# ZKI-PH-ImageAnalysis/seq2squiggle

Hardware: AMD Instinct MI355X
Metric: signal samples/sec at 5 kb reads (padded [chunks x 250] samples the predict path emits) (higher is better)
Workload: dtype f16x3

## Files before the change

### seq2squiggle_amd/csrc/s2s_device_h.h

```cpp
#pragma once
#include "s2s_device.h"

typedef _Float16 h8 __attribute__((ext_vector_type(8)));
typedef _Float16 h4 __attribute__((ext_vector_type(4)));

static constexpr float S2S_SHIFT_BIAS = 2.0f;
#define S2S_PF_FLOATS (1024 + 16 + 16)
#define S2S_Z2_FLOATS (256 + 64)
#define S2S_PROG_INTS 16
#define S2S_SV_FLOATS 960
#define WS_ADVP(n, bit) (ws += ((S2S_ABL & (bit)) ? 0 : (n)))
#ifndef S2S_NO_SB_ATT
#define SB_ATT() __builtin_amdgcn_sched_barrier(0)
#else
#define SB_ATT()
#endif
#ifndef S2S_NO_SB_GEMM
#define SB_GEMM() __builtin_amdgcn_sched_barrier(0)
#else
#define SB_GEMM()
#endif
#define MFMAH(a, b, c) __builtin_amdgcn_mfma_f32_16x16x32_f16((a), (b), (c), 0, 0, 0)
#ifndef S2S_MFMA_SPLIT
#define S2S_MFMA_SPLIT 0
// ... 5 lines not shown

__device__ __forceinline__ h8 as_h8(const f32x4 v) { return __builtin_bit_cast(h8, v); }

typedef _Float16 h2v __attribute__((ext_vector_type(2)));
template <bool LO = true>
__device__ __forceinline__ void split2(const float a, const float b, const float one, unsigned& hi, unsigned& lo) {
    unsigned hb = __builtin_bit_cast(unsigned, (h2v{(_Float16)a, (_Float16)b}));
    if (!LO) { hi = hb; lo = 0u; return; }
    asm("" : "+v"(hb));
    const h2v h = __builtin_bit_cast(h2v, hb);
    const h2v l = {(_Float16)__builtin_fmaf(a, one, -(float)h[0]), (_Float16)__builtin_fmaf(b, one, -(float)h[1])};
    hi = hb;
    lo = __builtin_bit_cast(unsigned, l);
}
template <bool LO = true>
__device__ __forceinline__ void exp_split4(const f32x4 s, const float one, unsigned& h0, unsigned& h1, unsigned& l0,
                                           unsigned& l1) {
    const float e0 = (S2S_ABL & 1) ? s[0] : __builtin_amdgcn_exp2f(s[0]), e1 = (S2S_ABL & 1) ? s[1] : __builtin_amdgcn_exp2f(s[1]);
    const float e2 = (S2S_ABL & 1) ? s[2] : __builtin_amdgcn_exp2f(s[2]), e3 = (S2S_ABL & 1) ? s[3] : __builtin_amdgcn_exp2f(s[3]);
    if (S2S_ABL & 2) {
        h0 = __float_as_uint(e0); l0 = __float_as_uint(e1); h1 = __float_as_uint(e2); l1 = __float_as_uint(e3);
        return;
    }
    split2<LO>(e0, e1, one, h0, l0);
    split2<LO>(e2, e3, one, h1, l1);
}
typedef unsigned uv4 __attribute__((ext_vector_type(4)));
typedef unsigned uv2 __attribute__((ext_vector_type(2)));
template <bool LO = true>
__device__ __forceinline__ HL split8(const f32x4 t0, const f32x4 t1, const float one) {
    unsigned h0, h1, h2, h3, l0, l1, l2, l3;
    split2<LO>(t0[0], t0[1], one, h0, l0);
    split2<LO>(t0[2], t0[3], one, h1, l1);
    split2<LO>(t1[0], t1[1], one, h2, l2);
    split2<LO>(t1[2], t1[3], one, h3, l3);
    HL o;
    o.hi = __builtin_bit_cast(h8, (uv4{h0, h1, h2, h3}));
    o.lo = __builtin_bit_cast(h8, (uv4{l0, l1, l2, l3}));
    return o;
}
template <bool LO = true>
__device__ __forceinline__ void split4(const f32x4 t, const float one, h4& hi, h4& lo) {
    unsigned h0, h1, l0, l1;
    split2<LO>(t[0], t[1], one, h0, l0);
    split2<LO>(t[2], t[3], one, h1, l1);
    hi = __builtin_bit_cast(h4, (uv2{h0, h1}));
    lo = __builtin_bit_cast(h4, (uv2{l0, l1}));
}

template <bool NATURAL = false>
__host__ __device__ constexpr int att32_key_at(const int p) {
    return NATURAL ? p : 16 * ((((p & 63) >> 2) - ((p >> 6) & 1)) & 15) + 4 * (p >> 6) + (p & 3);
}
template <int TV, bool NATURAL = false>
__device__ __forceinline__ void att32_mask_tile(f32x16& t, const int tile, const int h) {
#pragma unroll
    for (int r = 0; r < 16; ++r) {
        const int row = (r & 3) + 8 * (r >> 2);
        const bool p0 = att32_key_at<NATURAL>(32 * tile + row) >= TV, p1 = att32_key_at<NATURAL>(32 * tile + row + 4) >= TV;
        if (p0 && p1) t[r] = -__builtin_inff();
        else if (p1) t[r] = h ? -__builtin_inff() : t[r];
        else if (p0) t[r] = h ? t[r] : -__builtin_inff();
    }
}

template <int NQ, int WAVES, int NKT = 16> struct AttnLdsH {
    static_assert(NQ == 2 && NKT == 16, "the 32x32x16 attention core: 32 queries per wave, 256 keys");
    static constexpr int KEYS = 16 * NKT;
    static constexpr int K_BYTES = 8 * 2 * KEYS * 8 * 2;
    static constexpr int VS = KEYS + 8;
    static constexpr int V_BYTES = 8 * 16 * VS * 2;
    static constexpr int C_ROWS = 3;
    static constexpr int C_BYTES = C_ROWS * VS * 2;
    static constexpr int Q_WAVE_BYTES = NQ * 2 * 2 * 16 * 8 * 2;
    static constexpr int BYTES = K_BYTES + V_BYTES + C_BYTES + WAVES * Q_WAVE_BYTES;
};

template <int NQ, bool LO = true>
__device__ __forceinline__ void mm_unit_h(f32x4 (&acc)[NQ], const f32x4 (&f)[4], const HL (&x)[NQ][2]) {
#pragma unroll
    for (int kb = 0; kb < 2; ++kb) {
        const h8 wh = as_h8(f[2 * kb]), wl = as_h8(f[2 * kb + 1]);
#pragma unroll
        for (int q = 0; q < NQ; ++q) acc[q] = MFMAH(wh, x[q][kb].hi, acc[q]);
        if (LO) {
#pragma unroll
            for (int q = 0; q < NQ; ++q) acc[q] = MFMAH(wh, x[q][kb].lo, acc[q]);
#pragma unroll
            for (int q = 0; q < NQ; ++q) acc[q] = MFMAH(wl, x[q][kb].hi, acc[q]);
        }
    }
}

template <int NQ, bool LO = true>
__device__ __forceinline__ void mm_unit_h_t(f32x4 (&acc)[NQ], const f32x4 (&f)[4], const HL (&x)[NQ][2]) {
#pragma unroll
    for (int kb = 0; kb < 2; ++kb) {
        const h8 wh = as_h8(f[2 * kb]), wl = as_h8(f[2 * kb + 1]);
#pragma unroll
        for (int q = 0; q < NQ; ++q) acc[q] = MFMAH(x[q][kb].hi, wh, acc[q]);
        if (LO) {
#pragma unroll
            for (int q = 0; q < NQ; ++q) acc[q] = MFMAH(x[q][kb].lo, wh, acc[q]);
#pragma unroll
            for (int q = 0; q < NQ; ++q) acc[q] = MFMAH(x[q][kb].hi, wl, acc[q]);
        }
    }
}

template <int NQ>
__device__ __forceinline__ void linear64_h(const float* __restrict__ wu, const float* __restrict__ bias, int lane,
                                           const HL (&xb)[NQ][2], f32x4 (&y)[NQ][4]) {
    const int g = lane >> 4;
#pragma unroll
    for (int mt = 0; mt < 4; ++mt) {
        f32x4 f[4], t[NQ];
        load_unit(f, wu + mt * 1024 + lane * 4);
        const f32x4 b = ldg4(bias + 16 * mt + 4 * g);
// ... 11 lines not shown
    return fmaxf(__uint_as_float(t[0]), __uint_as_float(t[1]));
}
__device__ __forceinline__ float sum_h(float v) {
    const unsigned u = __float_as_uint(v);
    auto t = __builtin_amdgcn_permlane32_swap(u, u, false, false);
    return __uint_as_float(t[0]) + __uint_as_float(t[1]);
}
struct SelA { h8 a[2]; };
__device__ __forceinline__ SelA split_selectors(const int h) {
    const int row = threadIdx.x & 31, rho = row & 15;
    const int j = (rho & 3) + 4 * (rho >> 3);
    const unsigned w = (((rho >> 2) & 1) == h) ? ((j & 1) ? 0xBC000000u : 0x0000BC00u) : 0u;
    uv4 sel;
#pragma unroll
    for (int d = 0; d < 4; ++d) sel[d] = (j >> 1) == d ? w : 0u;
    const uv4 z = {0u, 0u, 0u, 0u};
    SelA o;
    o.a[0] = __builtin_bit_cast(h8, row < 16 ? sel : z);
    o.a[1] = __builtin_bit_cast(h8, row < 16 ? z : sel);
    return o;
}
template <bool LO>
__device__ __forceinline__ void pv_split_mfma(f32x16 sc, const h8 (&va)[2], const SelA& sel, f32x16& O) {
    unsigned hw[8];
#pragma unroll
    for (int r = 0; r < 16; ++r) sc[r] = __builtin_amdgcn_exp2f(sc[r]);
#pragma unroll
    for (int p = 0; p < 8; ++p) hw[p] = __builtin_bit_cast(unsigned, (h2v{(_Float16)sc[2 * p], (_Float16)sc[2 * p + 1]}));
    const h8 hb0 = __builtin_bit_cast(h8, (uv4{hw[0], hw[1], hw[2], hw[3]})), hb1 = __builtin_bit_cast(h8, (uv4{hw[4], hw[5], hw[6], hw[7]}));
    if (LO) {
        sc = MFMAW(sel.a[1], hb1, MFMAW(sel.a[0], hb0, sc));
        unsigned lw[8];
#pragma unroll
        for (int p = 0; p < 8; ++p) lw[p] = __builtin_bit_cast(unsigned, (h2v{(_Float16)sc[2 * p], (_Float16)sc[2 * p + 1]}));
        O = MFMAW(va[0], hb0, O);
        O = MFMAW(va[0], __builtin_bit_cast(h8, (uv4{lw[0], lw[1], lw[2], lw[3]})), O);
        O = MFMAW(va[1], hb1, O);
        O = MFMAW(va[1], __builtin_bit_cast(h8, (uv4{lw[4], lw[5], lw[6], lw[7]})), O);
    } else {
        O = MFMAW(va[0], hb0, O);
        O = MFMAW(va[1], hb1, O);
    }
}
template <int TV, bool SAFE, bool LO>
__device__ __forceinline__ void softmax_pv32(const _Float16* __restrict__ kp, const _Float16* __restrict__ kp2, const _Float16* __restrict__ vp,
                                             const h8 qb1, const h8 qb2, const float one, const int h, f32x16& O,
                                             [[maybe_unused]] const int layer = 0) {
    constexpr int NT = 8;
    const f32x16 zero16 = {0, 0, 0, 0, 0, 0, 0, 0, 0, 0, 0, 0, 0, 0, 0, 0};
    auto k_of = [&](const int t) { return *reinterpret_cast<const h8*>(kp + 32 * t * 8); };
    auto scores = [&](const h8 ka, const f32x16 c0) { return MFMAW(ka, qb2, MFMAW(ka, qb1, c0)); };
    O = zero16;
    auto v_of = [&](const int t, const int st) { return *reinterpret_cast<const h8*>(vp + 16 * (2 * t + st)); };
    auto mask_pass = [&](f32x16 (&t)[2], const int h2) {
        att32_mask_tile<TV>(t[0], 2 * h2, h);
        att32_mask_tile<TV>(t[1], 2 * h2 + 1, h);
    };
    auto pv = [&](const f32x16& t, const h8 (&va)[2]) {
#pragma unroll
        for (int st = 0; st < 2; ++st) {
            unsigned h0, h1, h2_, h3, l0, l1, l2, l3;
            exp_split4<LO>(f32x4{t[8 * st], t[8 * st + 1], t[8 * st + 2], t[8 * st + 3]}, one, h0, h1, l0, l1);
            exp_split4<LO>(f32x4{t[8 * st + 4], t[8 * st + 5], t[8 * st + 6], t[8 * st + 7]}, one, h2_, h3, l2, l3);
            O = MFMAW(va[st], __builtin_bit_cast(h8, (uv4{h0, h1, h2_, h3})), O);
            if (LO) O = MFMAW(va[st], __builtin_bit_cast(h8, (uv4{l0, l1, l2, l3})), O);
        }
    };
    f32x16 negm = zero16;
    h8 qb2m = qb2;
#if S2S_MFMA_SPLIT
    [[maybe_unused]] const SelA sel = split_selectors(h);
#endif
    if constexpr (!SAFE) {
#pragma unroll
        for (int h2 = 0; h2 < NT / 2; ++h2) {
            h8 ka[2], va[2][2];
#pragma unroll
            for (int i = 0; i < 2; ++i) {
                ka[i] = k_of(2 * h2 + i);
                va[i][0] = v_of(2 * h2 + i, 0); va[i][1] = v_of(2 * h2 + i, 1);
            }
            SB_ATT();
            h8 kb[2];
#pragma unroll
            for (int i = 0; i < 2; ++i) kb[i] = *reinterpret_cast<const h8*>(kp2 + (2 * h2 + i) * (h ? 0 : 32 * 8));
            f32x16 sc[2];
#pragma unroll
            for (int i = 0; i < 2; ++i) sc[i] = h2 == 0 ? MFMAW(ka[i], qb1, zero16) : MFMAW(kb[i], qb2m, MFMAW(ka[i], qb1, zero16));
            mask_pass(sc, h2);
            if (h2 == 0) {
                float mh = sc[0][0];
#pragma unroll
                for (int i = 0; i < 2; ++i)
#pragma unroll
                    for (int r = 0; r < 16; ++r) mh = fmaxf(mh, sc[i][r]);
                const float nm = -(max_h(mh) + S2S_SHIFT_BIAS);
                const _Float16 nh = (_Float16)nm;
                const unsigned pk = __builtin_bit_cast(unsigned, (h2v{nh, (_Float16)(nm - (float)nh)}));
                uv4 q2 = __builtin_bit_cast(uv4, qb2);
                q2[0] = h ? pk : q2[0];
                qb2m = __builtin_bit_cast(h8, q2);
#pragma unroll
                for (int i = 0; i < 2; ++i) sc[i] = MFMAW(kb[i], qb2m, sc[i]);
            }
#ifdef S2S_TILEHIST
#pragma unroll
            for (int i = 0; i < 2; ++i) {
                float m16[2];
#pragma unroll
                for (int st = 0; st < 2; ++st) {
                    float m = sc[i][8 * st];
#pragma unroll
                    for (int r = 1; r < 8; ++r) m = fmaxf(m, sc[i][8 * st + r]);
#pragma unroll
                    for (int o = 32; o > 0; o >>= 1) m = fmaxf(m, __shfl_xor(m, o, 64));
                    m16[st] = m + S2S_SHIFT_BIAS;
                }
                auto bin = [](const float t) { return t > 0.0f ? 63 : (-t >= 62.0f ? 62 : (int)(-t)); };
                if ((threadIdx.x & 63) == 0) {
                    atomicAdd(&s2s_hist_lds[(layer * 2 + 0) * 64 + bin(fmaxf(m16[0], m16[1]))], 1u);
                    atomicAdd(&s2s_hist_lds[(layer * 2 + 1) * 64 + bin(m16[0])], 1u);
                    atomicAdd(&s2s_hist_lds[(layer * 2 + 1) * 64 + bin(m16[1])], 1u);
                }
            }
#endif
#if S2S_MFMA_SPLIT
#pragma unroll
            for (int i = 0; i < 2; ++i) pv_split_mfma<LO>(sc[i], va[i], sel, O);
#else
#pragma unroll
            for (int i = 0; i < 2; ++i)
#pragma unroll
                for (int st = 0; st < 2; ++st) {
                    unsigned h0, h1, h2_, h3, l0, l1, l2, l3;
                    exp_split4<LO>(f32x4{sc[i][8 * st], sc[i][8 * st + 1], sc[i][8 * st + 2], sc[i][8 * st + 3]}, one, h0, h1, l0, l1);
                    exp_split4<LO>(f32x4{sc[i][8 * st + 4], sc[i][8 * st + 5], sc[i][8 * st + 6], sc[i][8 * st + 7]}, one, h2_, h3, l2, l3);
                    O = MFMAW(va[i][st], __builtin_bit_cast(h8, (uv4{h0, h1, h2_, h3})), O);
                    if (LO) O = MFMAW(va[i][st], __builtin_bit_cast(h8, (uv4{l0, l1, l2, l3})), O);
                }
#endif
        }
    } else {
        float m = 0.0f;
#pragma unroll
        for (int h2 = 0; h2 < NT / 2; ++h2) {
            h8 ka[2], va[2][2];
#pragma unroll
            for (int i = 0; i < 2; ++i) {
                ka[i] = k_of(2 * h2 + i);
                va[i][0] = v_of(2 * h2 + i, 0); va[i][1] = v_of(2 * h2 + i, 1);
            }
            f32x16 sc[2];
#pragma unroll
            for (int i = 0; i < 2; ++i) sc[i] = scores(ka[i], negm);
            mask_pass(sc, h2);
            float mh = sc[0][0];
#pragma unroll
            for (int i = 0; i < 2; ++i)
#pragma unroll
                for (int r = 0; r < 16; ++r) mh = fmaxf(mh, sc[i][r]);
            mh = max_h(mh);
            const float delta = (h2 == 0) ? mh : fmaxf(mh, 0.0f);
            if (h2 > 0) O *= __builtin_amdgcn_exp2f(-delta);
            m += delta;
#pragma unroll
            for (int r = 0; r < 16; ++r) negm[r] = -m;
#pragma unroll
            for (int i = 0; i < 2; ++i) { sc[i] -= delta; pv(sc[i], va[i]); }
        }
    }
}
template <int TV, bool LO>
__device__ __forceinline__ void softmax_pv32_online(const _Float16* __restrict__ kp, const _Float16* __restrict__ kp2, const _Float16* __restrict__ vp,
                                                    const h8 qb1, const h8 qb2, const float one, const int h, f32x16& O) {
    constexpr int NT = 8;
    const f32x16 zero16 = {0, 0, 0, 0, 0, 0, 0, 0, 0, 0, 0, 0, 0, 0, 0, 0};
    auto k_of = [&](const int t) { return *reinterpret_cast<const h8*>(kp + 32 * t * 8); };
    auto v_of = [&](const int t, const int st) { return *reinterpret_cast<const h8*>(vp + 16 * (2 * t + st)); };
    O = zero16;
    h8 qb2m = qb2;
#if S2S_MFMA_SPLIT
    const SelA sel = split_selectors(h);
#endif
    float m = 0.0f;
#pragma unroll
    for (int h2 = 0; h2 < NT / 2; ++h2) {
        h8 ka[2], kb[2], va[2][2];
#pragma unroll
        for (int i = 0; i < 2; ++i) {
            ka[i] = k_of(2 * h2 + i);
            kb[i] = *reinterpret_cast<const h8*>(kp2 + (2 * h2 + i) * (h ? 0 : 32 * 8));
            va[i][0] = v_of(2 * h2 + i, 0); va[i][1] = v_of(2 * h2 + i, 1);
        }
        SB_ATT();
        f32x16 sc[2];
#pragma unroll
        for (int i = 0; i < 2; ++i) sc[i] = MFMAW(ka[i], qb1, zero16);
        att32_mask_tile<TV, true>(sc[0], 2 * h2, h);
        att32_mask_tile<TV, true>(sc[1], 2 * h2 + 1, h);
        float mh = sc[0][0];
#pragma unroll
        for (int i = 0; i < 2; ++i)
#pragma unroll
            for (int r = 0; r < 16; ++r) mh = fmaxf(mh, sc[i][r]);
        mh = max_h(mh);
        const float nm = -(h2 == 0 ? mh : fmaxf(m, mh));
        const _Float16 nh = (_Float16)(-__builtin_ceilf(-nm));
        const unsigned pk = __builtin_bit_cast(unsigned, (h2v{nh, (_Float16)0.0f}));
        uv4 q2 = __builtin_bit_cast(uv4, qb2);
        q2[0] = h ? pk : q2[0];
        qb2m = __builtin_bit_cast(h8, q2);
        const float m_enc = -(float)nh;
        if (h2 > 0) {
            const float f = __builtin_amdgcn_exp2f(m - m_enc);
#pragma unroll
            for (int r = 0; r < 9; ++r) O[r] *= f;
        }
        m = m_enc;
#pragma unroll
        for (int i = 0; i < 2; ++i) sc[i] = MFMAW(kb[i], qb2m, sc[i]);
#if S2S_MFMA_SPLIT
#pragma unroll
        for (int i = 0; i < 2; ++i) pv_split_mfma<LO>(sc[i], va[i], sel, O);
#else
#pragma unroll
        for (int i = 0; i < 2; ++i)
#pragma unroll
            for (int st = 0; st < 2; ++st) {
                unsigned h0, h1, h2_, h3, l0, l1, l2, l3;
                exp_split4<LO>(f32x4{sc[i][8 * st], sc[i][8 * st + 1], sc[i][8 * st + 2], sc[i][8 * st + 3]}, one, h0, h1, l0, l1);
                exp_split4<LO>(f32x4{sc[i][8 * st + 4], sc[i][8 * st + 5], sc[i][8 * st + 6], sc[i][8 * st + 7]}, one, h2_, h3, l2, l3);
                O = MFMAW(va[i][st], __builtin_bit_cast(h8, (uv4{h0, h1, h2_, h3})), O);
                if (LO) O = MFMAW(va[i][st], __builtin_bit_cast(h8, (uv4{l0, l1, l2, l3})), O);
            }
#endif
    }
}
template <class G> __device__ __forceinline__ void att32_consts(char* __restrict__ lds, const int tid, const int nthreads) {
    _Float16* cr = reinterpret_cast<_Float16*>(lds + G::K_BYTES + G::V_BYTES);
    for (int i = tid; i < G::C_ROWS * G::VS; i += nthreads)
        cr[i] = (i < G::VS || (i >= 2 * G::VS && i < 3 * G::VS && ((i - 2 * G::VS) & 7) < 2)) ? (_Float16)1.0f : (_Float16)0.0f;
}

__device__ __forceinline__ const _Float16* zeros_row2(const float* sv_lds) {
    const unsigned a = (unsigned)(size_t)(sv_lds + S2S_SV_FLOATS + S2S_PROG_INTS);
    return reinterpret_cast<const _Float16*>(sv_lds + S2S_SV_FLOATS + S2S_PROG_INTS) + (((4u * 16u - (a & 255u)) & 255u) >> 1);
}

__device__ __forceinline__ void prio_balance(int* __restrict__ prog, const int wave) {
    const int lane = threadIdx.x & 63;
    int mine = prog[wave] + 1;
    if (lane == 0) prog[wave] = mine;
    const int theirs = __builtin_amdgcn_readfirstlane(prog[wave ^ 4]);
    mine = __builtin_amdgcn_readfirstlane(mine);
    if (mine <= theirs) __builtin_amdgcn_s_setprio(3); else __builtin_amdgcn_s_setprio(0);
}

template <bool LO>
__device__ __forceinline__ void load_unit_h(f32x4 (&f)[4], const float* __restrict__ ws) {
    if (LO) {
#pragma unroll
        for (int i = 0; i < 4; ++i) f[i] = ldg4(ws + i * 256);
    } else {
        f[0] = ldg4(ws); f[2] = ldg4(ws + 256);
        f[1] = f32x4{0, 0, 0, 0}; f[3] = f32x4{0, 0, 0, 0};
    }
}

template <int NQ, int WAVES, int NKT, int TV, bool LO = true, bool EXACT = false>
__device__ __forceinline__ void fft_block_h(const float* __restrict__ W, const LayerOff L, f32x4 (&X)[NQ][4],
                                            char* __restrict__ lds, int qt0, int wave, int lane, const float one,
                                            [[maybe_unused]] unsigned long long* diag_buf = nullptr, const float* __restrict__ pf_src = nullptr,
                                            float* __restrict__ pf_dst = nullptr, float* __restrict__ sv_lds = nullptr) {
    using G = AttnLdsH<NQ, WAVES, NKT>;
    constexpr bool SV = (WAVES == 8);
    auto svp = [&](const int off) -> const float* {
        if constexpr (SV) return sv_lds + (off - L.bq_nat); else return W + off;
    };
    const int sv_i = wave * 64 + lane;
    f32x4 svv = f32x4{0, 0, 0, 0};
    if (SV && sv_i < S2S_SV_FLOATS / 4) svv = ldg4(W + L.bq_nat + 4 * sv_i);
    const int g = lane >> 4, c = lane & 15;
    DIAG_DECL;
    _Float16* __restrict__ Kl = reinterpret_cast<_Float16*>(lds);
    _Float16* __restrict__ Vl = reinterpret_cast<_Float16*>(lds + G::K_BYTES);
    _Float16* __restrict__ Ql = reinterpret_cast<_Float16*>(lds + G::K_BYTES + G::V_BYTES + G::C_BYTES + wave * G::Q_WAVE_BYTES);
    constexpr int UF = LO ? 1024 : 512;
    const float* ws = W + (LO ? L.stream_h : L.stream_f) + lane * 4;
    f32x4 fa[4], fb[4];
    load_unit_h<LO>(fa, ws); WS_ADVP(UF, 2048);

    HL xb[NQ][2];
#pragma unroll
    for (int q = 0; q < NQ; ++q) { xb[q][0] = split8<LO>(X[q][0], X[q][1], one); xb[q][1] = split8<LO>(X[q][2], X[q][3], one); }

    if (!(S2S_ABL & 4)) block_sync<WAVES == 1>();
    DIAG_STAMP(0);
    if (SV && sv_i < S2S_SV_FLOATS / 4) *reinterpret_cast<f32x4*>(sv_lds + 4 * sv_i) = svv;
    f32x4 bk_n = ldg4(W + L.bk_nat + 4 * g);
    float bv_n = W[L.bv + c];
#pragma unroll 1
    for (int p = 0; p < 4; ++p) {
        if (S2S_ABL & 4096) { for (int i = 0; i < 4; ++i) fb[i] = fa[i]; } else load_unit_h<LO>(fb, ws);
        WS_ADVP(UF, 2048);
        const f32x4 bk = bk_n;
        const float bv = bv_n;
        bk_n = ldg4(W + L.bk_nat + 16 * (p < 3 ? p + 1 : 3) + 4 * g);
        bv_n = W[L.bv + 16 * (p < 3 ? p + 1 : 3) + c];
        SB_GEMM();
        f32x4 ak[NQ], av[NQ];
#pragma unroll
        for (int q = 0; q < NQ; ++q) { ak[q] = bk; av[q] = f32x4{bv, bv, bv, bv}; }
        if (!((S2S_ABL & (1 << 22)) && pf_src == nullptr)) mm_unit_h<NQ, LO>(ak, fa, xb);
        SB_GEMM();
        if (!(S2S_ABL & 4096) || p == 3) load_unit_h<LO>(fa, ws);
        WS_ADVP(UF, 2048);
        SB_GEMM();
        if (!((S2S_ABL & (1 << 22)) && pf_src == nullptr)) mm_unit_h_t<NQ, LO>(av, fb, xb);
        const int head = 2 * p + (g >> 1), d0 = 4 * (g & 1);
        const int vrow = (2 * p + (c >> 3)) * 16 + (c & 7);
#pragma unroll
        for (int q = 0; q < NQ; ++q) {
            const int T = qt0 + q;
            const int key = EXACT ? 16 * T + c : 64 * (c >> 2) + 4 * ((T + ((c >> 2) & 1)) & 15) + (c & 3);
            h4 hi, lo;
            split4<LO>(ak[q], one, hi, lo);
            *reinterpret_cast<h4*>(Kl + ((head * 2 + 0) * G::KEYS + key) * 8 + d0) = hi;
            *reinterpret_cast<h4*>(Kl + ((head * 2 + 1) * G::KEYS + key) * 8 + d0) = lo;
            split4<LO>(av[q], one, hi, lo);
            const int Tr = (T + (g & 1)) & 15;
            const int vcol = EXACT ? 16 * T + 8 * (g & 1) + 4 * ((g >> 1) & 1)
                                   : 16 * (4 * g + (Tr >> 2)) + 8 * (Tr & 1) + 4 * ((Tr >> 1) & 1);
            *reinterpret_cast<h4*>(Vl + vrow * G::VS + vcol) = hi;
            *reinterpret_cast<h4*>(Vl + (vrow + 8) * G::VS + vcol) = lo;
        }
    }
    DIAG_STAMP(1);
    if (!(S2S_ABL & 4)) block_sync<WAVES == 1>();
    DIAG_STAMP(2);
    f32x4 acc[NQ][4];
#pragma unroll
    for (int mt = 0; mt < 4; ++mt) {
        const f32x4 b = ldg4(svp(L.bfc) + 16 * mt + 4 * g);
#pragma unroll
        for (int q = 0; q < NQ; ++q) acc[q][mt] = X[q][mt] + b;
    }

#pragma unroll 1
    for (int u = 0; u < 2; ++u) {
        f32x4 opair[2][NQ];
#pragma unroll
        for (int pp = 0; pp < 2; ++pp) {
            const int p = 2 * u + pp;
            if (pp == 0) { load_unit_h<LO>(fb, ws); WS_ADVP(UF, 8192); } else { load_unit_h<LO>(fa, ws); WS_ADVP(UF, 8192); }
            const f32x4 bq = ldg4(svp(L.bq_nat) + 16 * p + 4 * g);
            SB_GEMM();
            f32x4 qa[NQ];
#pragma unroll
            for (int q = 0; q < NQ; ++q) qa[q] = bq;
            if (!((S2S_ABL & (1 << 22)) && pf_src == nullptr)) { if (pp == 0) mm_unit_h<NQ, LO>(qa, fa, xb); else mm_unit_h<NQ, LO>(qa, fb, xb); }
            SB_GEMM();
#pragma unroll
            for (int q = 0; q < NQ; ++q) {
                h4 hi, lo;
                split4<LO>(qa[q], one, hi, lo);
                *reinterpret_cast<h4*>(Ql + ((((g >> 1) * NQ + q) * 2 + 0) * 16 + c) * 8 + 4 * (g & 1)) = hi;
                *reinterpret_cast<h4*>(Ql + ((((g >> 1) * NQ + q) * 2 + 1) * 16 + c) * 8 + 4 * (g & 1)) = lo;
            }
            const int hl = lane >> 5, n = lane & 31;
            const _Float16* const crow = Vl + 8 * 16 * G::VS;
            const _Float16* const zrow2 = zeros_row2(sv_lds);
#pragma unroll
            for (int hh = 0; hh < 2; ++hh) {
                const int head = 2 * p + hh;
                if constexpr (WAVES == 8) prio_balance(reinterpret_cast<int*>(sv_lds + S2S_SV_FLOATS), wave);
                const _Float16* qrow = Ql + (((hh * NQ + (n >> 4)) * 2 + 0) * 16 + (n & 15)) * 8;
                const h8 qb1 = *reinterpret_cast<const h8*>(qrow);
                const h8 qb2 = *reinterpret_cast<const h8*>(hl ? crow + G::VS : qrow + 16 * 8);
                const _Float16* kp = Kl + ((head * 2 + hl) * G::KEYS + n) * 8;
                const _Float16* kp2 = hl ? crow + 2 * G::VS : kp;
                const _Float16* vp = (n < 16 ? Vl + (head * 16 + n) * G::VS : n == 16 ? crow : (n >= 20 && n < 28) ? zrow2 : crow + G::VS) + 8 * hl;
                f32x16 O;
                float lsum;
                if constexpr (EXACT) {
                    softmax_pv32_online<TV, LO>(kp, kp2, vp, qb1, qb2, one, hl, O);
                    lsum = sum_h(O[8]);
                } else {
                    softmax_pv32<TV, false, LO>(kp, kp2, vp, qb1, qb2, one, hl, O, pf_src ? 1 : 0);
                    lsum = sum_h(O[8]);
// ... 336 lines not shown
```

### seq2squiggle_amd/csrc/s2s_hip.hip

```cpp
#include "s2s_device.h"
#include "s2s_device_h.h"
#include "s2s_generic.h"
#include "s2s_generic_h.h"
#include "../../include/s2s_hip.h"
#include "s2s_event_fixed.h"
#define S2S_DTW_KERNELS
#include "s2s_dtw.h"
#include "s2s_sdtw.h"
#include "s2s_resquiggle.h"
#include "s2s_segment.h"
#include "s2s_eventalign.h"
#include "s2s_chunk.h"

#include <cctype>
#include <cstdio>
#include <cstdlib>
#include <cstring>
#include <immintrin.h>
#include <map>
#include <mutex>
#include <string>
#include <vector>

template <int NQ>
// ... 225 lines not shown
        HL Sb[NQ][2];
#pragma unroll
        for (int q = 0; q < NQ; ++q) { Sb[q][0] = split8(X[q][0], X[q][1], one); Sb[q][1] = split8(X[q][2], X[q][3], one); }
        float sig[NQ], cq[NQ], rq[NQ];
#pragma unroll
        for (int q = 0; q < NQ; ++q) { cq[q] = 1.0f; rq[q] = 1.0f; }
        auto head = [&](const MlpOff m, float (&out)[NQ]) {
            f32x4 hid[NQ][4];
            linear64_h<NQ>(W + m.w0h, W + m.b0, lane, Sb, hid);
            head_out<NQ>(W, m, hid, lane, out);
        };
        head(M.noise, sig);
        if (P.duration_sampling) { head(M.conc, cq); head(M.rate, rq); }
        FDIAG(4);
        front_dwell<NQ, EVAL>(io, P, sig, cq, rq, dbg, lane);
    }
#pragma unroll
    for (int ft = 0; ft < 4; ++ft) {
        const f32x4 pe = ldg4(W + M.pe_enc + c * 64 + 16 * ft + 4 * g);
#pragma unroll
        for (int q = 0; q < NQ; ++q) X[q][ft] += pe;
    }
    FDIAG(5);
#pragma unroll 1
    for (int l = 0; l < M.enc_layers; ++l) {
        const LayerOff L = M.enc[l];
        const float* const wl = W + L.stream_h;
        f32x4 acc[NQ][4];
        HL x1b[NQ][2];
        enc_attention_h<NQ>(W, L, wl, X, acc, lane, one);
        FDIAG(2);
        enc_ffn_begin_h<NQ>(W, L, acc, X, x1b, lane, one);
        enc_ffn_half_h<NQ>(W, L, wl + 16 * 1024, 0, x1b, X, lane, one);
        enc_ffn_half_h<NQ>(W, L, wl + 32 * 1024, 2, x1b, X, lane, one);
        layer_norm64<NQ, true>(X, W + L.ln2g, W + L.ln2b, g);
        FDIAG(3);
    }
    front_store<NQ>(io, dbg, X, lane, true);
}

#define DEC_WAVES 8
#define DEC_NQ 2
#define DEC_WPS (DEC_WAVES / 4)
#define DEC_NKT 16
static constexpr int DEC_LDS_F32 = AttnLds<DEC_NKT>::BYTES;
static constexpr int DEC_LDS_H = AttnLdsH<DEC_NQ, DEC_WAVES, DEC_NKT>::BYTES;


struct GatherRaw {
    f32x4 e[DEC_NQ][4], pe[DEC_NQ][4];
    float sg[DEC_NQ];
    int idx[DEC_NQ];
};
__device__ __forceinline__ void dec_gather_issue(const ModelDev& M, const float* __restrict__ W, const float* __restrict__ slot,
                                                 const int wave, const int lane, GatherRaw& R) {
    const int g = lane >> 4, c = lane & 15;
    const int qt0 = DEC_NQ * wave;
    int cum[16];
    {
        const int dv = reinterpret_cast<const int*>(slot + 1040)[c];
        int run = 0;
#pragma unroll
        for (int j = 0; j < 16; ++j) {
            const int dj = __builtin_amdgcn_readlane(dv, j);
            run += dj < S2S_T_DEC + 1 ? dj : S2S_T_DEC + 1;
            cum[j] = run;
        }
    }
#pragma unroll
    for (int q = 0; q < DEC_NQ; ++q) {
        const int t = 16 * (qt0 + q) + c;
        int idx = 0;
#pragma unroll
        for (int j = 0; j < 16; ++j) idx += (cum[j] <= t) ? 1 : 0;
        R.idx[q] = idx;
        const int row = idx < 16 ? idx : 0;
        const float* er = slot + row * 64 + 4 * g;
        const float* pr = W + M.pe_dec + (t < S2S_T_DEC ? t : 0) * 64 + 4 * g;
#pragma unroll
        for (int ft = 0; ft < 4; ++ft) { R.e[q][ft] = ldg4(er + 16 * ft); R.pe[q][ft] = ldg4(pr + 16 * ft); }
        R.sg[q] = slot[1024 + row];
    }
}
__device__ __forceinline__ void dec_gather_finish(const GatherRaw& R, const int wave, const int lane, f32x4 (&X)[DEC_NQ][4],
                                                  float (&sig_ext)[DEC_NQ]) {
    const int c = lane & 15;
#pragma unroll
    for (int q = 0; q < DEC_NQ; ++q) {
        const int t = 16 * (DEC_NQ * wave + q) + c;
        const bool live = R.idx[q] < 16, real = t < S2S_T_DEC;
#pragma unroll
        for (int ft = 0; ft < 4; ++ft)
            X[q][ft] = real ? ((live ? R.e[q][ft] : f32x4{0, 0, 0, 0}) + R.pe[q][ft]) : f32x4{0, 0, 0, 0};
        sig_ext[q] = live ? R.sg[q] : 0.0f;
    }
}

__device__ __forceinline__ void dec_override(const float* __restrict__ dec_in, const long long dbg_idx, const int wave, const int lane,
                                             f32x4 (&X)[DEC_NQ][4]) {
    const int g = lane >> 4, c = lane & 15;
#pragma unroll
    for (int q = 0; q < DEC_NQ; ++q) {
        const int t = 16 * (DEC_NQ * wave + q) + c;
#pragma unroll
        for (int ft = 0; ft < 4; ++ft)
            X[q][ft] = t < S2S_T_DEC ? ldg4(dec_in + (dbg_idx * S2S_T_DEC + t) * 64 + 16 * ft + 4 * g) : f32x4{0, 0, 0, 0};
    }
}

template <int MODE, bool EXACT = false>
__device__ __forceinline__ void dec_blocks(const ModelDev& M, const float* __restrict__ W, f32x4 (&X)[DEC_NQ][4],
                                           char* __restrict__ lds_raw, const int wave, const int lane, const float one,
                                           unsigned long long* diag, const float* __restrict__ next_slot = nullptr) {
    const int qt0 = DEC_NQ * wave;
#pragma unroll 1
    for (int l = 0; l < M.dec_layers; ++l) {
        float* const slot_lds = reinterpret_cast<float*>(lds_raw + DEC_LDS_H), *const sv_lds = slot_lds + S2S_SLOT_FLOATS;
        if (MODE == 1) fft_block_h<DEC_NQ, DEC_WAVES, DEC_NKT, S2S_T_DEC, true, EXACT>(W, M.dec[l], X, lds_raw, qt0, wave, lane, one, diag,
                                                                          l == M.dec_layers - 1 ? next_slot : nullptr, slot_lds, sv_lds);
        else if (MODE == 3) fft_block_h<DEC_NQ, DEC_WAVES, DEC_NKT, S2S_T_DEC, false, EXACT>(W, M.dec[l], X, lds_raw, qt0, wave, lane, one, diag,
                                                                                      nullptr, slot_lds, sv_lds);
        else           fft_block<DEC_NQ, DEC_NKT, S2S_T_DEC>(W, M.dec[l], X, reinterpret_cast<float*>(lds_raw), qt0, lane, diag);
    }
}

__device__ __forceinline__ void dec_project(const ModelDev& M, const float* __restrict__ W, const f32x4 (&X)[DEC_NQ][4],
                                            const float (&sig_ext)[DEC_NQ], const int lane, float& ys, float& se) {
    const int g = lane >> 4;
    f32x4 wo[4];
#pragma unroll
    for (int ft = 0; ft < 4; ++ft) wo[ft] = ldg4(W + M.out_w + 16 * ft + 4 * g);
    const float bo = W[M.out_b];
    ys = 0.0f; se = 0.0f;
#pragma unroll
    for (int q = 0; q < DEC_NQ; ++q) {
        float part = 0.0f;
#pragma unroll
        for (int ft = 0; ft < 4; ++ft)
#pragma unroll
            for (int r = 0; r < 4; ++r) part += X[q][ft][r] * wo[ft][r];
        const float v = relu1(sum_g(part) + bo);
        if (g == q) { ys = v; se = sig_ext[q]; }
    }
}

__device__ __forceinline__ void dec_emit(const ModelDev& M, const float ys, const float se, const unsigned long long chunk,
                                         const ParamsDev& P, const float* __restrict__ inj_z01, float* __restrict__ out_signal,
                                         const DebugDev& dbg, const long long dbg_idx, const int wave, const int lane) {
    const int g = lane >> 4, c = lane & 15;
    const int t = 16 * (DEC_NQ * wave + g) + c;
    float y = __fmul_rn(ys, M.scale);
    if (g < DEC_NQ && t < S2S_T_DEC) {
        if (dbg.y_scaled) dbg.y_scaled[dbg_idx * S2S_T_DEC + t] = ys;
        if (P.noise_std > 0.0f) {
            float z;
            if (inj_z01) {
                z = inj_z01[t];
            } else {
                const u32x4 r = philox4x32_10((unsigned)chunk, (unsigned)(chunk >> 32),
                                              (unsigned)t | (S2S_KIND_NOISE << 16), 0, P.seed_lo, P.seed_hi);
                z = box_muller(r.x, r.y);
            }
            if (dbg.z01) dbg.z01[dbg_idx * S2S_T_DEC + t] = z;
            const float sd = P.noise_sampling
                                 ? __fmul_rn(__fmul_rn(fmaxf(se, P.min_noise), P.noise_std), M.scale)
                                 : P.noise_std;
            if (y != 0.0f) y = mul_then_add(z, sd, y);
        }
        store_stream(out_signal + t, fmaxf(y, 0.0f));
    }
}

template <int MODE> struct Fused {
    static constexpr int FMODE = (MODE == 3) ? 1 : MODE;
    static constexpr int FNQ = (FMODE == 1) ? 2 : 1;
    static constexpr int GROUP = DEC_WAVES * FNQ;
    static constexpr bool PF = (MODE == 1);
    static constexpr int LDS = (MODE == 0) ? DEC_LDS_F32 : DEC_LDS_H + (S2S_SLOT_FLOATS + S2S_SV_FLOATS + S2S_PROG_INTS + S2S_Z2_FLOATS) * 4;
    static_assert(LDS + S2S_STATIC_LDS_BYTES + 16 <= 160 * 1024, "LDS per workgroup: dynamic + the static arrays in front of it");
    static_assert(FMODE == 1 || DEC_WAVES * FrontLdsF32::BYTES <= LDS, "the f32 frontend waves' K/V images share the decoder's LDS");
};
#define S2S_MAX_GROUP (2 * DEC_WAVES)
template <int MODE, bool TEST, bool EXACT = false>
__global__ __launch_bounds__(DEC_WAVES * 64, DEC_WPS) void s2s_fused_kernel(
    const ModelDev M, const float* __restrict__ W, const uint8_t* __restrict__ bases,
    const long long* __restrict__ chunk_start, const uint8_t* __restrict__ n_valid, int n_chunks, long long first_chunk,
    ParamsDev P, const float* __restrict__ inj_g_, const float* __restrict__ inj_zdw_, const float* __restrict__ inj_z01_,
    float* __restrict__ handoff, int* __restrict__ out_dur, float* __restrict__ out_signal, DebugDev dbg_, long long dbg_base) {
    using F = Fused<MODE>;
    const float* const inj_g = TEST ? inj_g_ : nullptr;
    const float* const inj_zdw = TEST ? inj_zdw_ : nullptr;
    const float* const inj_z01 = TEST ? inj_z01_ : nullptr;
    DebugDev dbg = dbg_;
    if (!TEST) { dbg = DebugDev{}; dbg.diag = dbg_.diag; dbg.stats = dbg_.stats; }
    extern __shared__ __attribute__((aligned(16))) char lds_raw[];
    const int wave = __builtin_amdgcn_readfirstlane(threadIdx.x >> 6);
    const int lane = threadIdx.x & 63;
    const int nb = S2S_T_ENC + M.k - 1;
    if constexpr (MODE != 0) att32_consts<AttnLdsH<DEC_NQ, DEC_WAVES, DEC_NKT>>(lds_raw, threadIdx.x, DEC_WAVES * 64);
    if constexpr (MODE != 0) {
        if (threadIdx.x < S2S_PROG_INTS + S2S_Z2_FLOATS)
            reinterpret_cast<int*>(lds_raw + DEC_LDS_H + (S2S_SLOT_FLOATS + S2S_SV_FLOATS) * 4)[threadIdx.x] = 0;
    }
    if (threadIdx.x == 0) {
        const unsigned long long c0 = __builtin_readcyclecounter(), r0 = __builtin_amdgcn_s_memrealtime();
        s2s_stats_lds[0] = 0;
        s2s_stats_lds[4] = (unsigned)c0; s2s_stats_lds[5] = (unsigned)(c0 >> 32);
        s2s_stats_lds[6] = (unsigned)r0; s2s_stats_lds[7] = (unsigned)(r0 >> 32);
    }
#ifdef S2S_TILEHIST
    for (int i = threadIdx.x; i < 2 * 2 * 64; i += DEC_WAVES * 64) s2s_hist_lds[i] = 0;
#endif
#ifdef S2S_DIAG
    for (int i = threadIdx.x; i < 8 * S2S_DIAG_SLOTS; i += DEC_WAVES * 64) s2s_diag_lds[i] = 0;
    const unsigned long long diag_c0 = __builtin_readcyclecounter(), diag_r0 = __builtin_amdgcn_s_memrealtime();
    __syncthreads();
#endif
    float* const slot0 = handoff + (size_t)blockIdx.x * S2S_MAX_GROUP * S2S_SLOT_FLOATS;
    const int lo = (int)((long long)blockIdx.x * n_chunks / gridDim.x), hi = (int)((long long)(blockIdx.x + 1) * n_chunks / gridDim.x);
#pragma unroll 1
    for (int g0 = lo; g0 < hi; g0 += F::GROUP) {
        const int n_here = hi - g0 < F::GROUP ? hi - g0 : F::GROUP;
        float one = 1.0f;
        asm volatile("" : "+s"(one));
        DIAG_DECL;
        __syncthreads();
        {
            int lnf = lane;
            asm volatile("" : "+v"(lnf));
            auto chunk_of = [&](const int j, const int j_filler) {
                const bool live = j < n_here;
                const int b = g0 + (live ? j : j_filler);
                return FrontChunk{chunk_start ? bases + chunk_start[b] : bases + (size_t)b * nb, n_valid[b],
                                  (unsigned long long)(first_chunk + b), inj_g ? inj_g + (size_t)b * 16 : nullptr,
                                  inj_zdw ? inj_zdw + (size_t)b * 16 : nullptr, slot0 + j * S2S_SLOT_FLOATS,
                                  out_dur + (size_t)b * 16, dbg_base + b, live};
            };
            if constexpr (F::FMODE == 1) {
                if (n_here > DEC_WAVES) {
                    const FrontChunk io[2] = {chunk_of(2 * wave, 2 * wave), chunk_of(2 * wave + 1, 2 * wave)};
                    if (2 * wave < n_here) frontend_h16<2>(M, W, io, P, dbg, lnf, one);
                } else {
                    const FrontChunk io[1] = {chunk_of(wave, 0)};
                    if (wave < n_here) frontend_h16<1>(M, W, io, P, dbg, lnf, one);
                }
            } else {
                const FrontChunk io[1] = {chunk_of(wave, 0)};
                if (wave < n_here) frontend_f32(M, W, io, P, lds_raw + wave * FrontLdsF32::BYTES, dbg, lnf);
            }
        }
        __syncthreads();
        DIAG_STAMP(7);
        f32x4 X[DEC_NQ][4];
        float sig_ext[DEC_NQ];
        {
            int lg = lane;
            asm volatile("" : "+v"(lg));
            GatherRaw R;
            dec_gather_issue(M, W, slot0, wave, lg, R);
            dec_gather_finish(R, wave, lg, X, sig_ext);
            if (TEST && dbg.dec_in) dec_override(dbg.dec_in, dbg_base + g0, wave, lg, X);
        }
        DIAG_STAMP(8);
#pragma unroll 1
        for (int j = 0; j < ((S2S_ABL & 65536) ? 0 : n_here); ++j) {
            const int b = g0 + j;
            const float* next = slot0 + (j + 1 < n_here ? j + 1 : j) * S2S_SLOT_FLOATS;
            dec_blocks<MODE, EXACT>(M, W, X, lds_raw, wave, lane, one, dbg.diag, F::PF ? next : nullptr);
            DIAG_STAMP(15);
            int ln = lane;
            asm volatile("" : "+v"(ln));
            float ys, se;
            dec_project(M, W, X, sig_ext, ln, ys, se);
            GatherRaw R;
            if constexpr (F::PF) dec_gather_issue(M, W, reinterpret_cast<const float*>(lds_raw + DEC_LDS_H), wave, ln, R);
            else                 dec_gather_issue(M, W, next, wave, ln, R);
            dec_emit(M, ys, se, (unsigned long long)(first_chunk + b), P, inj_z01 ? inj_z01 + (size_t)b * S2S_T_DEC : nullptr,
                     out_signal + (size_t)b * S2S_T_DEC, dbg, dbg_base + b, wave, ln);
            dec_gather_finish(R, wave, ln, X, sig_ext);
            if (TEST && dbg.dec_in) dec_override(dbg.dec_in, dbg_base + g0 + (j + 1 < n_here ? j + 1 : j), wave, ln, X);
            DIAG_STAMP(9);
        }
    }
#ifdef S2S_DIAG
    DIAG_COUNT(16, __builtin_readcyclecounter() - diag_c0);
    DIAG_COUNT(17, __builtin_amdgcn_s_memrealtime() - diag_r0);
    DIAG_COUNT(18, 1ull);
    __syncthreads();
    if (dbg.diag)
        for (int i = threadIdx.x; i < 8 * S2S_DIAG_SLOTS; i += DEC_WAVES * 64)
            if (s2s_diag_lds[i]) atomicAdd(dbg.diag + i, s2s_diag_lds[i]);
#endif
    __syncthreads();
#ifdef S2S_TILEHIST
    if (dbg.diag)
        for (int i = threadIdx.x; i < 2 * 2 * 64; i += DEC_WAVES * 64)
            if (s2s_hist_lds[i]) atomicAdd(dbg.diag + i, (unsigned long long)s2s_hist_lds[i]);
#endif
    if (threadIdx.x == 0 && dbg.stats) {
        const unsigned long long c0 = ((unsigned long long)s2s_stats_lds[5] << 32) | s2s_stats_lds[4];
        const unsigned long long r0 = ((unsigned long long)s2s_stats_lds[7] << 32) | s2s_stats_lds[6];
        if (s2s_stats_lds[0]) atomicAdd(dbg.stats + S2S_STAT_REDO, (unsigned long long)s2s_stats_lds[0]);
        atomicAdd(dbg.stats + S2S_STAT_CYCLES, __builtin_readcyclecounter() - c0);
        atomicAdd(dbg.stats + S2S_STAT_TICKS, __builtin_amdgcn_s_memrealtime() - r0);
        atomicAdd(dbg.stats + S2S_STAT_WGS, 1ull);
    }
}

template <int MODE, bool EXACT>
__global__ __launch_bounds__(DEC_WAVES * 64, DEC_WPS) void s2s_eval_kernel(
    const ModelDev M, const float* __restrict__ W, const uint8_t* __restrict__ kmers, const int* __restrict__ dwell, int n_chunks,
    ParamsDev P, float* __restrict__ handoff, float* __restrict__ y, DebugDev dbg_) {
    using F = Fused<MODE>;
    extern __shared__ __attribute__((aligned(16))) char lds_raw[];
    const int wave = __builtin_amdgcn_readfirstlane(threadIdx.x >> 6);
    const int lane = threadIdx.x & 63;
    if constexpr (MODE != 0) att32_consts<AttnLdsH<DEC_NQ, DEC_WAVES, DEC_NKT>>(lds_raw, threadIdx.x, DEC_WAVES * 64);
    if constexpr (MODE != 0) {
        if (threadIdx.x < S2S_PROG_INTS + S2S_Z2_FLOATS)
            reinterpret_cast<int*>(lds_raw + DEC_LDS_H + (S2S_SLOT_FLOATS + S2S_SV_FLOATS) * 4)[threadIdx.x] = 0;
    }
    if (threadIdx.x == 0) s2s_stats_lds[0] = 0;
    DebugDev dbg{};
    dbg.sigma = dbg_.sigma; dbg.conc = dbg_.conc; dbg.rate = dbg_.rate;
    float* const slot0 = handoff + (size_t)blockIdx.x * S2S_MAX_GROUP * S2S_SLOT_FLOATS;
    const int lo = (int)((long long)blockIdx.x * n_chunks / gridDim.x), hi = (int)((long long)(blockIdx.x + 1) * n_chunks / gridDim.x);
    const int kb = S2S_T_ENC * M.k;
#pragma unroll 1
    for (int g0 = lo; g0 < hi; g0 += F::GROUP) {
        const int n_here = hi - g0 < F::GROUP ? hi - g0 : F::GROUP;
        float one = 1.0f;
        asm volatile("" : "+s"(one));
        __syncthreads();
        {
            int lnf = lane;
            asm volatile("" : "+v"(lnf));
            auto chunk_of = [&](const int j, const int j_filler) {
                const bool live = j < n_here;
                const int b = g0 + (live ? j : j_filler);
                return FrontChunk{kmers + (size_t)b * kb, S2S_T_ENC, (unsigned long long)b, nullptr, nullptr, slot0 + j * S2S_SLOT_FLOATS,
                                  const_cast<int*>(dwell) + (size_t)b * S2S_T_ENC, (long long)b, live};
            };
            if constexpr (F::FMODE == 1) {
                if (n_here > DEC_WAVES) {
                    const FrontChunk io[2] = {chunk_of(2 * wave, 2 * wave), chunk_of(2 * wave + 1, 2 * wave)};
                    if (2 * wave < n_here) frontend_h16<2, true>(M, W, io, P, dbg, lnf, one);
                } else {
                    const FrontChunk io[1] = {chunk_of(wave, 0)};
                    if (wave < n_here) frontend_h16<1, true>(M, W, io, P, dbg, lnf, one);
                }
            } else {
                const FrontChunk io[1] = {chunk_of(wave, 0)};
                if (wave < n_here) frontend_f32<true>(M, W, io, P, lds_raw + wave * FrontLdsF32::BYTES, dbg, lnf);
            }
        }
        __syncthreads();
        f32x4 X[DEC_NQ][4];
        float sig_ext[DEC_NQ];
        {
            int lg = lane;
            asm volatile("" : "+v"(lg));
            GatherRaw R;
            dec_gather_issue(M, W, slot0, wave, lg, R);
            dec_gather_finish(R, wave, lg, X, sig_ext);
        }
#pragma unroll 1
        for (int j = 0; j < n_here; ++j) {
            const int b = g0 + j;
            const float* next = slot0 + (j + 1 < n_here ? j + 1 : j) * S2S_SLOT_FLOATS;
            dec_blocks<MODE, EXACT>(M, W, X, lds_raw, wave, lane, one, nullptr, F::PF ? next : nullptr);
            int ln = lane;
            asm volatile("" : "+v"(ln));
            float ys, se;
            dec_project(M, W, X, sig_ext, ln, ys, se);
            GatherRaw R;
            if constexpr (F::PF) dec_gather_issue(M, W, reinterpret_cast<const float*>(lds_raw + DEC_LDS_H), wave, ln, R);
            else                 dec_gather_issue(M, W, next, wave, ln, R);
            {
                const int g = ln >> 4, t = 16 * (DEC_NQ * wave + g) + (ln & 15);
                if (g < DEC_NQ && t < S2S_T_DEC) store_stream(y + (size_t)b * S2S_T_DEC + t, ys);
            }
            dec_gather_finish(R, wave, ln, X, sig_ext);
        }
    }
}

__global__ __launch_bounds__(256) void s2s_eval_loss_kernel(const float* __restrict__ y, const float* __restrict__ target,
                                                            const float* __restrict__ sigma, const float* __restrict__ stdev,
                                                            const float* __restrict__ conc, const float* __restrict__ rate,
                                                            const int* __restrict__ dwell, int B, int te, int ts, float* __restrict__ out_loss) {
    const long long b = (long long)blockIdx.x * 4 + (threadIdx.x >> 6);
    const int lane = threadIdx.x & 63;
    if (b >= B) return;
    float se = 0.0f;
    for (int t = lane; t < ts; t += 64) {
        const float e = y[b * ts + t] - target[b * ts + t];
        se += e * e;
    }
    float nll = 0.0f, ne = 0.0f;
    if (lane < te) {
        const long long i = b * te + lane;
        const int dv = dwell[i];
        const float x = dv == 0 ? 1.0f : (float)(dv < 0 ? -dv : dv);
        const float a = conc[i], r = rate[i];
        const float am1 = a - 1.0f;
        const float lp = a * logf(r) + (am1 == 0.0f ? 0.0f : am1 * logf(x)) - r * x - lgammaf(a);
        nll = -lp;
        const float e = stdev[i] - sigma[i];
        ne = e * e;
    }
    se = gen_wave_sum(se);
    nll = gen_wave_sum(nll);
    ne = gen_wave_sum(ne);
    if (lane == 0) { out_loss[b * 3 + 0] = se; out_loss[b * 3 + 1] = nll; out_loss[b * 3 + 2] = ne; }
}

template <int TD>
__global__ __launch_bounds__(256) void s2s_count_kernel(const float* __restrict__ signal, int B, int* __restrict__ counts, int ts) {
    const int T = TD ? TD : ts;
    const int b = blockIdx.x * 4 + (threadIdx.x >> 6), lane = threadIdx.x & 63;
    if (b >= B) return;
    int n = 0;
    for (int t = lane; t < T; t += 64) n += signal[(size_t)b * T + t] != 0.0f;
#pragma unroll
    for (int o = 32; o > 0; o >>= 1) n += __shfl_xor(n, o, 64);
    if (lane == 0) counts[b] = n;
}

__global__ __launch_bounds__(1024) void s2s_scan_kernel(const int* __restrict__ counts, int B, long long* __restrict__ offs) {
    __shared__ long long wsum[16];
    __shared__ long long carry_s;
    const int tid = threadIdx.x, lane = tid & 63, w = tid >> 6;
    if (tid == 0) carry_s = 0;
    __syncthreads();
    for (int base = 0; base < B; base += 8192) {
// ... 1972 lines not shown
```

Before: 720.7 million.

## Replace per-tile attention padding masks with zeroed V columns and cloned phantom rows

Removes the per-score-tile -inf masking of phantom keys (positions at or beyond the real decoder length) from every softmax pass. Instead the padded query rows are filled as clones of the last real timestep, the V columns for phantom keys are zeroed in LDS, and the ones-row used for the softmax denominator drops those keys. Phantom keys then add nothing to either the numerator or the denominator, which saves the select instructions in the hot attention loop. The cost is a small extra LDS write pass on the last time tile. The scheme relies on the phantom keys having finite scores, which cloning the real rows is meant to guarantee.

```diff
diff --git a/seq2squiggle_amd/csrc/s2s_device_h.h b/seq2squiggle_amd/csrc/s2s_device_h.h
--- a/seq2squiggle_amd/csrc/s2s_device_h.h
+++ b/seq2squiggle_amd/csrc/s2s_device_h.h
@@ -81,18 +81,10 @@
 __host__ __device__ constexpr int att32_key_at(const int p) {
     return NATURAL ? p : 16 * ((((p & 63) >> 2) - ((p >> 6) & 1)) & 15) + 4 * (p >> 6) + (p & 3);
 }
-template <int TV, bool NATURAL = false>
-__device__ __forceinline__ void att32_mask_tile(f32x16& t, const int tile, const int h) {
-#pragma unroll
-    for (int r = 0; r < 16; ++r) {
-        const int row = (r & 3) + 8 * (r >> 2);
-        const bool p0 = att32_key_at<NATURAL>(32 * tile + row) >= TV, p1 = att32_key_at<NATURAL>(32 * tile + row + 4) >= TV;
-        if (p0 && p1) t[r] = -__builtin_inff();
-        else if (p1) t[r] = h ? -__builtin_inff() : t[r];
-        else if (p0) t[r] = h ? t[r] : -__builtin_inff();
-    }
-}
-
+template <bool NATURAL>
+__host__ __device__ constexpr int att32_key_at_vpos(const int i) {
+    return att32_key_at<NATURAL>(16 * (i >> 4) + 4 * ((i >> 3) & 1) + (i & 3) + 8 * ((i >> 2) & 1));
+}
 template <int NQ, int WAVES, int NKT = 16> struct AttnLdsH {
     static_assert(NQ == 2 && NKT == 16, "the 32x32x16 attention core: 32 queries per wave, 256 keys");
     static constexpr int KEYS = 16 * NKT;
@@ -210,10 +202,6 @@
     auto scores = [&](const h8 ka, const f32x16 c0) { return MFMAW(ka, qb2, MFMAW(ka, qb1, c0)); };
     O = zero16;
     auto v_of = [&](const int t, const int st) { return *reinterpret_cast<const h8*>(vp + 16 * (2 * t + st)); };
-    auto mask_pass = [&](f32x16 (&t)[2], const int h2) {
-        att32_mask_tile<TV>(t[0], 2 * h2, h);
-        att32_mask_tile<TV>(t[1], 2 * h2 + 1, h);
-    };
     auto pv = [&](const f32x16& t, const h8 (&va)[2]) {
 #pragma unroll
         for (int st = 0; st < 2; ++st) {
@@ -245,7 +233,6 @@
             f32x16 sc[2];
 #pragma unroll
             for (int i = 0; i < 2; ++i) sc[i] = h2 == 0 ? MFMAW(ka[i], qb1, zero16) : MFMAW(kb[i], qb2m, MFMAW(ka[i], qb1, zero16));
-            mask_pass(sc, h2);
             if (h2 == 0) {
                 float mh = sc[0][0];
 #pragma unroll
@@ -311,7 +298,6 @@
             f32x16 sc[2];
 #pragma unroll
             for (int i = 0; i < 2; ++i) sc[i] = scores(ka[i], negm);
-            mask_pass(sc, h2);
             float mh = sc[0][0];
 #pragma unroll
             for (int i = 0; i < 2; ++i)
@@ -354,8 +340,6 @@
         f32x16 sc[2];
 #pragma unroll
         for (int i = 0; i < 2; ++i) sc[i] = MFMAW(ka[i], qb1, zero16);
-        att32_mask_tile<TV, true>(sc[0], 2 * h2, h);
-        att32_mask_tile<TV, true>(sc[1], 2 * h2 + 1, h);
         float mh = sc[0][0];
 #pragma unroll
         for (int i = 0; i < 2; ++i)
@@ -394,10 +378,11 @@
 #endif
     }
 }
-template <class G> __device__ __forceinline__ void att32_consts(char* __restrict__ lds, const int tid, const int nthreads) {
+template <class G, int TV, bool NATURAL>
+__device__ __forceinline__ void att32_consts(char* __restrict__ lds, const int tid, const int nthreads) {
     _Float16* cr = reinterpret_cast<_Float16*>(lds + G::K_BYTES + G::V_BYTES);
     for (int i = tid; i < G::C_ROWS * G::VS; i += nthreads)
-        cr[i] = (i < G::VS || (i >= 2 * G::VS && i < 3 * G::VS && ((i - 2 * G::VS) & 7) < 2)) ? (_Float16)1.0f : (_Float16)0.0f;
+        cr[i] = ((i < G::VS && !(i < G::KEYS && att32_key_at_vpos<NATURAL>(i) >= TV)) || (i >= 2 * G::VS && i < 3 * G::VS && ((i - 2 * G::VS) & 7) < 2)) ? (_Float16)1.0f : (_Float16)0.0f;
 }
 
 __device__ __forceinline__ const _Float16* zeros_row2(const float* sv_lds) {
@@ -493,6 +478,16 @@
             *reinterpret_cast<h4*>(Vl + (vrow + 8) * G::VS + vcol) = lo;
         }
     }
+    if constexpr (TV < 16 * NKT) {
+        static_assert(TV % 2 == 0 && TV >= 16 * (NKT - 1), "phantom keys: whole pairs of halves, all in the last time tile");
+        if (qt0 + NQ == NKT) {
+#pragma unroll
+            for (int r = 0; r < 8 * 16; r += 64)
+#pragma unroll
+                for (int i = 0; i < G::KEYS; i += 2)
+                    if (att32_key_at_vpos<EXACT>(i) >= TV) *reinterpret_cast<unsigned*>(Vl + (r + lane) * G::VS + i) = 0u;
+        }
+    }
     DIAG_STAMP(1);
     if (!(S2S_ABL & 4)) block_sync<WAVES == 1>();
     DIAG_STAMP(2);
diff --git a/seq2squiggle_amd/csrc/s2s_hip.hip b/seq2squiggle_amd/csrc/s2s_hip.hip
--- a/seq2squiggle_amd/csrc/s2s_hip.hip
+++ b/seq2squiggle_amd/csrc/s2s_hip.hip
@@ -301,6 +301,7 @@
     float sg[DEC_NQ];
     int idx[DEC_NQ];
 };
+template <bool CLONE>
 __device__ __forceinline__ void dec_gather_issue(const ModelDev& M, const float* __restrict__ W, const float* __restrict__ slot,
                                                  const int wave, const int lane, GatherRaw& R) {
     const int g = lane >> 4, c = lane & 15;
@@ -318,7 +319,7 @@
     }
 #pragma unroll
     for (int q = 0; q < DEC_NQ; ++q) {
-        const int t = 16 * (qt0 + q) + c;
+        const int t0 = 16 * (qt0 + q) + c, t = (CLONE && t0 >= S2S_T_DEC) ? S2S_T_DEC - 1 : t0;
         int idx = 0;
 #pragma unroll
         for (int j = 0; j < 16; ++j) idx += (cum[j] <= t) ? 1 : 0;
@@ -331,13 +332,14 @@
         R.sg[q] = slot[1024 + row];
     }
 }
+template <bool CLONE>
 __device__ __forceinline__ void dec_gather_finish(const GatherRaw& R, const int wave, const int lane, f32x4 (&X)[DEC_NQ][4],
                                                   float (&sig_ext)[DEC_NQ]) {
     const int c = lane & 15;
 #pragma unroll
     for (int q = 0; q < DEC_NQ; ++q) {
         const int t = 16 * (DEC_NQ * wave + q) + c;
-        const bool live = R.idx[q] < 16, real = t < S2S_T_DEC;
+        const bool live = R.idx[q] < 16, real = CLONE || t < S2S_T_DEC;
 #pragma unroll
         for (int ft = 0; ft < 4; ++ft)
             X[q][ft] = real ? ((live ? R.e[q][ft] : f32x4{0, 0, 0, 0}) + R.pe[q][ft]) : f32x4{0, 0, 0, 0};
@@ -345,12 +347,13 @@
     }
 }
 
+template <bool CLONE>
 __device__ __forceinline__ void dec_override(const float* __restrict__ dec_in, const long long dbg_idx, const int wave, const int lane,
                                              f32x4 (&X)[DEC_NQ][4]) {
     const int g = lane >> 4, c = lane & 15;
 #pragma unroll
     for (int q = 0; q < DEC_NQ; ++q) {
-        const int t = 16 * (DEC_NQ * wave + q) + c;
+        const int t0 = 16 * (DEC_NQ * wave + q) + c, t = (CLONE && t0 >= S2S_T_DEC) ? S2S_T_DEC - 1 : t0;
 #pragma unroll
         for (int ft = 0; ft < 4; ++ft)
             X[q][ft] = t < S2S_T_DEC ? ldg4(dec_in + (dbg_idx * S2S_T_DEC + t) * 64 + 16 * ft + 4 * g) : f32x4{0, 0, 0, 0};
@@ -446,7 +449,7 @@
     const int wave = __builtin_amdgcn_readfirstlane(threadIdx.x >> 6);
     const int lane = threadIdx.x & 63;
     const int nb = S2S_T_ENC + M.k - 1;
-    if constexpr (MODE != 0) att32_consts<AttnLdsH<DEC_NQ, DEC_WAVES, DEC_NKT>>(lds_raw, threadIdx.x, DEC_WAVES * 64);
+    if constexpr (MODE != 0) att32_consts<AttnLdsH<DEC_NQ, DEC_WAVES, DEC_NKT>, S2S_T_DEC, EXACT>(lds_raw, threadIdx.x, DEC_WAVES * 64);
     if constexpr (MODE != 0) {
         if (threadIdx.x < S2S_PROG_INTS + S2S_Z2_FLOATS)
             reinterpret_cast<int*>(lds_raw + DEC_LDS_H + (S2S_SLOT_FLOATS + S2S_SV_FLOATS) * 4)[threadIdx.x] = 0;
@@ -506,9 +509,9 @@
             int lg = lane;
             asm volatile("" : "+v"(lg));
             GatherRaw R;
-            dec_gather_issue(M, W, slot0, wave, lg, R);
-            dec_gather_finish(R, wave, lg, X, sig_ext);
-            if (TEST && dbg.dec_in) dec_override(dbg.dec_in, dbg_base + g0, wave, lg, X);
+            dec_gather_issue<MODE != 0>(M, W, slot0, wave, lg, R);
+            dec_gather_finish<MODE != 0>(R, wave, lg, X, sig_ext);
+            if (TEST && dbg.dec_in) dec_override<MODE != 0>(dbg.dec_in, dbg_base + g0, wave, lg, X);
         }
         DIAG_STAMP(8);
 #pragma unroll 1
@@ -522,12 +525,12 @@
             float ys, se;
             dec_project(M, W, X, sig_ext, ln, ys, se);
             GatherRaw R;
-            if constexpr (F::PF) dec_gather_issue(M, W, reinterpret_cast<const float*>(lds_raw + DEC_LDS_H), wave, ln, R);
-            else                 dec_gather_issue(M, W, next, wave, ln, R);
+            if constexpr (F::PF) dec_gather_issue<MODE != 0>(M, W, reinterpret_cast<const float*>(lds_raw + DEC_LDS_H), wave, ln, R);
+            else                 dec_gather_issue<MODE != 0>(M, W, next, wave, ln, R);
             dec_emit(M, ys, se, (unsigned long long)(first_chunk + b), P, inj_z01 ? inj_z01 + (size_t)b * S2S_T_DEC : nullptr,
                      out_signal + (size_t)b * S2S_T_DEC, dbg, dbg_base + b, wave, ln);
-            dec_gather_finish(R, wave, ln, X, sig_ext);
-            if (TEST && dbg.dec_in) dec_override(dbg.dec_in, dbg_base + g0 + (j + 1 < n_here ? j + 1 : j), wave, ln, X);
+            dec_gather_finish<MODE != 0>(R, wave, ln, X, sig_ext);
+            if (TEST && dbg.dec_in) dec_override<MODE != 0>(dbg.dec_in, dbg_base + g0 + (j + 1 < n_here ? j + 1 : j), wave, ln, X);
             DIAG_STAMP(9);
         }
     }
@@ -564,7 +567,7 @@
     extern __shared__ __attribute__((aligned(16))) char lds_raw[];
     const int wave = __builtin_amdgcn_readfirstlane(threadIdx.x >> 6);
     const int lane = threadIdx.x & 63;
-    if constexpr (MODE != 0) att32_consts<AttnLdsH<DEC_NQ, DEC_WAVES, DEC_NKT>>(lds_raw, threadIdx.x, DEC_WAVES * 64);
+    if constexpr (MODE != 0) att32_consts<AttnLdsH<DEC_NQ, DEC_WAVES, DEC_NKT>, S2S_T_DEC, EXACT>(lds_raw, threadIdx.x, DEC_WAVES * 64);
     if constexpr (MODE != 0) {
         if (threadIdx.x < S2S_PROG_INTS + S2S_Z2_FLOATS)
             reinterpret_cast<int*>(lds_raw + DEC_LDS_H + (S2S_SLOT_FLOATS + S2S_SV_FLOATS) * 4)[threadIdx.x] = 0;
@@ -610,8 +613,8 @@
             int lg = lane;
             asm volatile("" : "+v"(lg));
             GatherRaw R;
-            dec_gather_issue(M, W, slot0, wave, lg, R);
-            dec_gather_finish(R, wave, lg, X, sig_ext);
+            dec_gather_issue<MODE != 0>(M, W, slot0, wave, lg, R);
+            dec_gather_finish<MODE != 0>(R, wave, lg, X, sig_ext);
         }
 #pragma unroll 1
         for (int j = 0; j < n_here; ++j) {
@@ -623,13 +626,13 @@
             float ys, se;
             dec_project(M, W, X, sig_ext, ln, ys, se);
             GatherRaw R;
-            if constexpr (F::PF) dec_gather_issue(M, W, reinterpret_cast<const float*>(lds_raw + DEC_LDS_H), wave, ln, R);
-            else                 dec_gather_issue(M, W, next, wave, ln, R);
+            if constexpr (F::PF) dec_gather_issue<MODE != 0>(M, W, reinterpret_cast<const float*>(lds_raw + DEC_LDS_H), wave, ln, R);
+            else                 dec_gather_issue<MODE != 0>(M, W, next, wave, ln, R);
             {
                 const int g = ln >> 4, t = 16 * (DEC_NQ * wave + g) + (ln & 15);
                 if (g < DEC_NQ && t < S2S_T_DEC) store_stream(y + (size_t)b * S2S_T_DEC + t, ys);
             }
-            dec_gather_finish(R, wave, ln, X, sig_ext);
+            dec_gather_finish<MODE != 0>(R, wave, ln, X, sig_ext);
         }
     }
 }
```

New measurement: 722.6 million, median of 6. Within noise of the previous version (+0.3%).
